# nateraw/stable-diffusion-videos

Hardware: AMD Instinct MI355X
Metric: interpolated frames/sec (512x512, 50 DDIM steps) (higher is better)
Workload: dtype bf16; 1 GPU; sd14 walk, 2 prompts, 640 interpolated frames (5 steps x 128 frames x 1 GPU; BASELINE config 2 names 60 frames - this is the same walk with more frames, see `walk_60_frames` for the literal one), 512x512, 50 DDIM steps, CFG 7.5; batch_size=128, frames=640, parallelism=frame-sharded dp1, hipgraph=True

## Files before the change

### include/sdv_hip.h

```cpp
#ifndef SDV_HIP_H
#define SDV_HIP_H

#include <stdint.h>

#ifdef __cplusplus
extern "C" {
#endif

typedef uint16_t sdv_bf16;

#define SDV_OK 0
#define SDV_ERR_ARG (-1)
#define SDV_ERR_LAUNCH (-2)

const char* sdv_last_error(void);
int sdv_abi_version(void);

typedef struct sdv_gemm_args {
    const sdv_bf16* X;
    const sdv_bf16* X2;
    const sdv_bf16* W;
    const float* bias;
    const sdv_bf16* R;
    sdv_bf16* C;
// ... 20 lines not shown
    uint8_t* out_u8;
    float* gn_out;
    int32_t gn_ld;
    int32_t split_k;
} sdv_gemm_args;

int sdv_gemm_bf16(const sdv_gemm_args* args, void* stream);
int sdv_gemm_stats_slots(const sdv_gemm_args* args);
int sdv_gemm_split_k(const sdv_gemm_args* args);

int sdv_gemm_set_persistent(int on);
int sdv_gemm_set_grid_limit(int n);
int sdv_rowstats_finalize(const float* partials, int64_t rows, int32_t slots, int32_t C, float eps, float* out, void* stream);

int sdv_ffn_geglu_bf16(const sdv_bf16* X, const float* ln_stats, int64_t M, int32_t C, int32_t ldx, const sdv_bf16* W1, const sdv_bf16* W1x,
                       const sdv_bf16* W2p, const float* bias2, sdv_bf16* out, int32_t ldo, void* stream);

int sdv_linear320_bf16(const sdv_bf16* X, int64_t M, int32_t ldx, const sdv_bf16* W, const sdv_bf16* Wx, int32_t N, const float* ln_stats,
                       const float* alpha, const sdv_bf16* R, int32_t ldr, sdv_bf16* out, int32_t ldo, float* stats_out, float eps,
                       sdv_bf16* Vt, int32_t ldvt, int32_t hw, void* stream);

int sdv_linear640_bf16(const sdv_bf16* X, int64_t M, int32_t ldx, const sdv_bf16* W, const sdv_bf16* Wx, int32_t N, const float* ln_stats,
                       const float* alpha, sdv_bf16* out, int32_t ldo, float* stats_out, float eps, void* stream);

int sdv_attention_bf16(const sdv_bf16* Q, const sdv_bf16* K, const sdv_bf16* Vt, sdv_bf16* O,
                       int32_t B, int32_t H, int32_t Lq, int32_t Lk, int32_t dh,
                       int32_t ldq, int32_t ldk, int32_t ldv, int32_t ldo, float scale, int32_t causal,
                       int32_t q_prescaled, int32_t v_rowmajor, void* stream);

int sdv_softmax_rows_bf16(sdv_bf16* S, int64_t rows, int32_t cols, int32_t ld, void* stream);
int sdv_softmax_rows_f32(const float* S, sdv_bf16* P, int64_t rows, int32_t cols, int32_t lds, int32_t ldp, void* stream);

int sdv_groupnorm_finalize(const float* P1, int32_t C1, int32_t ld1, int32_t bpi1, int32_t nrep1, int64_t rep_stride1,
                           const float* P2, int32_t C2, int32_t ld2, int32_t bpi2, int32_t nrep2, int64_t rep_stride2,
                           int32_t nimg, int32_t groups, int32_t splits, float* partials, void* stream);
int sdv_groupnorm_stats(const sdv_bf16* X, const sdv_bf16* X2, int32_t C1, int32_t C2, int32_t nimg,
                        int32_t HW, int32_t groups, int32_t splits, float* partials, void* stream);
int sdv_groupnorm_apply(const sdv_bf16* X, const sdv_bf16* X2, int32_t C1, int32_t C2, int32_t nimg,
                        int32_t HW, int32_t groups, int32_t splits, const float* partials,
                        const float* gamma, const float* beta, float eps, int32_t silu, sdv_bf16* Y,
                        void* stream);
int sdv_groupnorm_apply_fp8(const sdv_bf16* X, const sdv_bf16* X2, int32_t C1, int32_t C2, int32_t nimg,
                            int32_t HW, int32_t groups, int32_t splits, const float* partials,
                            const float* gamma, const float* beta, float eps, int32_t silu, uint8_t* Y8,
                            float q_scale, void* stream);
int sdv_groupnorm_fp8_set_saturation_counter(int32_t* counter);

int sdv_layernorm_bf16(const sdv_bf16* X, const float* gamma, const float* beta, float eps, int64_t rows,
                       int32_t C, sdv_bf16* Y, void* stream);

int sdv_conv3x3_cin_small(const sdv_bf16* X, const sdv_bf16* W , const float* bias,
                          sdv_bf16* Y, int32_t nimg, int32_t H, int32_t Wd, int32_t Cin, int32_t Cout,
                          int32_t circular, void* stream);
int sdv_im2col3x3_c4(const sdv_bf16* X, sdv_bf16* Y, int32_t nimg, int32_t H, int32_t Wd, int32_t circular, void* stream);

int sdv_latent_affine(const float* X, const float* Wpq , const float* bias, float in_scale,
                      sdv_bf16* Y, int64_t npix, int32_t C, void* stream);

int sdv_slerp_stats(const float* v0, const float* v1, int64_t n, double* stats, void* stream);
int sdv_slerp_batch(const float* v0, const float* v1, const double* stats, const float* T, int32_t nframes,
                    int32_t C, int32_t HW, int32_t to_hwc, float dot_threshold, float* out, void* stream);
int sdv_lerp_batch(const float* a, const float* b, const float* T, int32_t nframes, int64_t n,
                   float* out_f32, sdv_bf16* out_bf16, void* stream);

int sdv_cfg_ddim_step(const float* eps, float* latents, sdv_bf16* x2, const float* coefs,
                      const int32_t* step_ptr, const float* noise, float guidance, int32_t cfg,
                      int64_t n_per_batch , void* stream);
int sdv_cfg_multistep_step(const float* eps, float* latents, sdv_bf16* x2, float* hist, float* xsave, const float* table,
                           const int32_t* step_ptr, const float* noise, float guidance, int32_t cfg,
                           int64_t n_per_batch , void* stream);
int sdv_latents_to_unet_input(const float* latents, sdv_bf16* x2, int32_t cfg, int64_t n, void* stream);
int sdv_step_counter_add(int32_t* step_ptr, int32_t inc, void* stream);

int sdv_timestep_embedding(const float* timesteps, int32_t n, int32_t dim, int32_t flip_sin_to_cos,
                           float freq_shift, float* out, void* stream);
int sdv_linear_small(const float* x, const sdv_bf16* w, const float* b, const float* add, float* out,
                     int32_t M, int32_t N, int32_t K, int32_t silu_in, void* stream);

int sdv_nchw_to_nhwc_f32(const float* in, float* out, int32_t n, int32_t C, int32_t HW, void* stream);
int sdv_nhwc_to_nchw_f32(const float* in, float* out, int32_t n, int32_t C, int32_t HW, void* stream);
int sdv_f32_to_bf16(const float* in, sdv_bf16* out, int64_t n, void* stream);

int sdv_embed_tokens(const int64_t* ids, const float* tok , const float* pos , sdv_bf16* out,
                     int64_t n_tokens, int32_t L, int32_t D, int32_t vocab, void* stream);

int sdv_rgb_u8_to_bf16_c4(const uint8_t* in, sdv_bf16* out, int64_t npix, float scale, void* stream);
int sdv_axpby_bf16(const sdv_bf16* a, int32_t lda, const sdv_bf16* b, int32_t ldb, sdv_bf16* out, int32_t ldo,
                   int64_t rows, int32_t cols, float alpha, float beta, void* stream);

int sdv_clip_preprocess_patches(const uint8_t* frames, sdv_bf16* patches, int32_t n, int32_t H, int32_t W, int32_t S, int32_t P,
                                int32_t Kpad, const int32_t* x_off, const int32_t* x_cnt, const float* x_w, int32_t x_taps,
                                const int32_t* y_off, const int32_t* y_cnt, const float* y_w, int32_t y_taps,
                                const float* host_mean, const float* host_std, void* stream);
int sdv_safety_screen(const float* image_embeds, const float* concept_embeds, const float* special_care_embeds,
                      const float* concept_thr, const float* special_thr, int32_t n, int32_t D, int32_t n_concept,
                      int32_t n_special, uint8_t* frames, int64_t frame_bytes, int32_t* flags, float* scores, void* stream);

int sdv_jpeg_transform_u8(const uint8_t* frames, int32_t n, int32_t H, int32_t W, const uint16_t* qtab_luma,
                          const uint16_t* qtab_chroma, int16_t* coef, void* stream);
int sdv_jpeg_entropy_pack(const int16_t* coef, int32_t n, int32_t H, int32_t W, const uint8_t* header, int32_t header_len,
                          void* scratch, int64_t scratch_bytes, uint8_t* out, int64_t out_cap, int64_t* offsets, int64_t* needed,
                          void* stream);

int sdv_png_filter_u8(const uint8_t* frames, int32_t n, int32_t H, int32_t W, uint8_t* filtered, uint32_t* adler_rows, void* stream);
int sdv_png_deflate_pack(const uint8_t* filtered, const uint32_t* adler_rows, int32_t n, int32_t H, int32_t W, int32_t stripe_rows,
                         const uint8_t* header, int32_t header_len, void* scratch, int64_t scratch_bytes, uint8_t* out,
// ... 19 lines not shown
```

### stable_diffusion_videos_amd/build.py

```python
from __future__ import annotations

import os
import shutil
import subprocess
import sys
from concurrent.futures import ThreadPoolExecutor
from pathlib import Path

PKG = Path(__file__).resolve().parent
CSRC = PKG / "csrc"
INCLUDE = PKG.parent / "include"
LIBDIR = PKG / "lib"
OBJDIR = PKG / "lib" / "obj"
LIB = LIBDIR / "libsdv_hip.so"
ARCH = "gfx950"

FLAGS = ["--offload-arch=" + ARCH, "-O3", "-std=c++17", "-fPIC", "-Wno-unused-result", "-I", str(INCLUDE)]
FAST_MATH = {"sdv_gemm.hip", "sdv_attention.hip", "sdv_norm.hip", "sdv_ffn.hip"}
FAST_FLAGS = ["-ffast-math", "-fno-finite-math-only"]
EXTRA_FLAGS = {"sdv_attention.hip": ["-mllvm", "-amdgpu-mfma-vgpr-form"],
               "sdv_gemm.hip": ["-mllvm", "-amdgpu-mfma-vgpr-form", "-fno-slp-vectorize"],
               "sdv_ffn.hip": ["-fno-slp-vectorize"],
               "sdv_vision.hip": ["-fno-slp-vectorize"]}


def hipcc() -> str:
    exe = shutil.which("hipcc") or "/opt/rocm/bin/hipcc"
    if not Path(exe).exists():
        raise RuntimeError("hipcc not found: cannot build libsdv_hip.so")
    return exe


def sources():
    return sorted(CSRC.glob("*.hip"))


def _newest_dep() -> float:
    deps = list(CSRC.glob("*.h")) + list(INCLUDE.glob("*.h")) + [Path(__file__)]
    return max(p.stat().st_mtime for p in deps)


def _compile(src: Path, force: bool) -> Path:
    obj = OBJDIR / (src.stem + ".o")
    if (not force and obj.exists() and obj.stat().st_mtime >= src.stat().st_mtime
            and obj.stat().st_mtime >= _newest_dep()):
        return obj
    cmd = [hipcc(), *FLAGS, *(FAST_FLAGS if src.name in FAST_MATH else []), *EXTRA_FLAGS.get(src.name, []), "-c", str(src), "-o", str(obj)]
    r = subprocess.run(cmd, capture_output=True, text=True)
    if r.returncode != 0:
        raise RuntimeError(f"hipcc failed for {src.name}:\n{r.stdout}\n{r.stderr}")
    if r.stderr.strip():
        sys.stderr.write(r.stderr)
    return obj


def build(force: bool = False, verbose: bool = False) -> Path:
    OBJDIR.mkdir(parents=True, exist_ok=True)
    srcs = sources()
    if not srcs:
        raise RuntimeError(f"no .hip sources under {CSRC}")
    with ThreadPoolExecutor(max_workers=min(len(srcs), os.cpu_count() or 4)) as ex:
        objs = list(ex.map(lambda s: _compile(s, force), srcs))
    if force or not LIB.exists() or any(o.stat().st_mtime > LIB.stat().st_mtime for o in objs):
        cmd = [hipcc(), "--offload-arch=" + ARCH, "-shared", "-fPIC", *map(str, objs), "-o", str(LIB)]
        r = subprocess.run(cmd, capture_output=True, text=True)
        if r.returncode != 0:
            raise RuntimeError(f"link failed:\n{r.stdout}\n{r.stderr}")
    if verbose:
        print(f"built {LIB} ({LIB.stat().st_size >> 10} KiB) from {[s.name for s in srcs]}")
    return LIB


if __name__ == "__main__":
    build(force="--force" in sys.argv, verbose=True)
```

### stable_diffusion_videos_amd/csrc/sdv_norm.hip

```cpp
#include "sdv_common.h"

namespace {

struct GnGeom {
    int C, nchunk, CT, PT;
};
__device__ __forceinline__ GnGeom gn_geom(int C) {
    GnGeom g;
    g.C = C;
    g.nchunk = C >> 3;
    g.CT = g.nchunk < 256 ? g.nchunk : 256;
    g.PT = 256 / g.CT;
    return g;
}

__device__ __forceinline__ const uint16_t* gn_src(const uint16_t* X, const uint16_t* X2, int C1, int C2, long long pix,
                                                  int c0) {
    return c0 < C1 ? X + pix * C1 + c0 : X2 + pix * C2 + (c0 - C1);
}

__global__ __launch_bounds__(256) void gn_stats_kernel(const uint16_t* __restrict__ X, const uint16_t* __restrict__ X2,
                                                       int C1, int C2, int HW, int groups, int splits,
                                                       float* __restrict__ partials) {
    extern __shared__ __attribute__((aligned(16))) float sm[];
// ... 244 lines not shown
    const int sub = lane % LPR;
    const long long row = ((long long)blockIdx.x * 4 + (threadIdx.x >> 6)) * RPWV + lane / LPR;
    const bool live = row < rows;
    const uint16_t* x = X + (live ? row : 0) * C;
    bf16x8_raw raw[5];
#pragma unroll
    for (int i = 0; i < 5; ++i) raw[i] = *(const bf16x8_raw*)(x + (sub + LPR * i) * 8);
    float f[5][8];
    float s = 0.f;
#pragma unroll
    for (int i = 0; i < 5; ++i) {
        unpack8(raw[i], f[i]);
#pragma unroll
        for (int e = 0; e < 8; ++e) s += f[i][e];
    }
#pragma unroll
    for (int o = LPR / 2; o > 0; o >>= 1) s += __shfl_xor(s, o);
    const float mean = s / (float)C;
    float q = 0.f;
#pragma unroll
    for (int i = 0; i < 5; ++i)
#pragma unroll
        for (int e = 0; e < 8; ++e) {
            const float d = f[i][e] - mean;
            q += d * d;
        }
#pragma unroll
    for (int o = LPR / 2; o > 0; o >>= 1) q += __shfl_xor(q, o);
    const float rstd = rsqrtf(q / (float)C + eps);
    if (!live) return;
    uint16_t* y = Y + row * C;
#pragma unroll
    for (int i = 0; i < 5; ++i) {
        const int c0 = (sub + LPR * i) * 8;
        const float4 g0 = *(const float4*)(gamma + c0), g1 = *(const float4*)(gamma + c0 + 4);
        const float4 b0 = *(const float4*)(beta + c0), b1 = *(const float4*)(beta + c0 + 4);
        const float gg[8] = {g0.x, g0.y, g0.z, g0.w, g1.x, g1.y, g1.z, g1.w};
        const float bb[8] = {b0.x, b0.y, b0.z, b0.w, b1.x, b1.y, b1.z, b1.w};
        float o[8];
#pragma unroll
        for (int e = 0; e < 8; ++e) o[e] = (f[i][e] - mean) * rstd * gg[e] + bb[e];
        *(bf16x8_raw*)(y + c0) = pack8(o);
    }
}

}

namespace {
struct GnSrc {
    const float* P;
    int C, ld, bpi, nrep;
    long long rep_stride;
};
__global__ __launch_bounds__(256) void gn_finalize_kernel(GnSrc a, GnSrc b, int groups, int splits, float* __restrict__ partials) {
    extern __shared__ __attribute__((aligned(16))) float sm[];
    const int C = a.C + b.C, cpg = C / groups;
    const int img = blockIdx.x, split = blockIdx.y;
    for (int c = threadIdx.x; c < C; c += 256) {
        const GnSrc& s = c < a.C ? a : b;
        const int cc = c < a.C ? c : c - a.C;
        const int per = (s.bpi + splits - 1) / splits;
        const int k0 = split * per, k1 = k0 + per < s.bpi ? k0 + per : s.bpi;
        float s1 = 0.f, s2 = 0.f;
        for (int r = 0; r < s.nrep; ++r) {
            const float* base = s.P + ((r * s.rep_stride + (long long)img * s.bpi) * 2) * s.ld + cc;
            int k = k0;
            for (; k + 3 < k1; k += 4) {
                float t[8];
#pragma unroll
                for (int j = 0; j < 8; ++j) t[j] = base[(long long)(2 * k + j) * s.ld];
#pragma unroll
                for (int j = 0; j < 4; ++j) {
                    s1 += t[2 * j];
                    s2 += t[2 * j + 1];
                }
            }
            for (; k < k1; ++k) {
                s1 += base[(long long)(2 * k) * s.ld];
                s2 += base[(long long)(2 * k + 1) * s.ld];
            }
        }
        sm[2 * c] = s1;
        sm[2 * c + 1] = s2;
    }
    __syncthreads();
    if (threadIdx.x < groups) {
        float as = 0.f, aq = 0.f;
        for (int c = 0; c < cpg; ++c) {
            as += sm[2 * (threadIdx.x * cpg + c)];
            aq += sm[2 * (threadIdx.x * cpg + c) + 1];
        }
        float* out = partials + (((long long)img * splits + split) * groups + threadIdx.x) * 2;
        out[0] = as;
        out[1] = aq;
    }
}
}

extern "C" int sdv_groupnorm_finalize(const float* P1, int32_t C1, int32_t ld1, int32_t bpi1, int32_t nrep1, int64_t rep_stride1,
                                      const float* P2, int32_t C2, int32_t ld2, int32_t bpi2, int32_t nrep2, int64_t rep_stride2,
                                      int32_t nimg, int32_t groups, int32_t splits, float* partials, void* stream) {
    SDV_REQUIRE(P1 && partials && C1 > 0 && nimg > 0, "sdv_groupnorm_finalize: bad args");
    SDV_REQUIRE(C2 == 0 || P2, "sdv_groupnorm_finalize: C2 > 0 needs P2");
    const int C = C1 + C2;
    SDV_REQUIRE(groups > 0 && groups <= 64 && C % groups == 0, "sdv_groupnorm_finalize: bad groups %d for C=%d", groups, C);
    SDV_REQUIRE(bpi1 > 0 && nrep1 > 0 && (C2 == 0 || (bpi2 > 0 && nrep2 > 0)) && splits > 0 && splits <= 64, "sdv_groupnorm_finalize: bad block geometry");
    SDV_REQUIRE((size_t)C * 8 <= 64 * 1024, "sdv_groupnorm_finalize: C=%d too large", C);
    GnSrc a{P1, C1, ld1, bpi1, nrep1, rep_stride1};
    GnSrc b{C2 ? P2 : P1, C2, C2 ? ld2 : ld1, C2 ? bpi2 : 1, C2 ? nrep2 : 1, C2 ? rep_stride2 : 0};
    hipLaunchKernelGGL(gn_finalize_kernel, dim3(nimg, splits), dim3(256), (size_t)C * 8, (hipStream_t)stream, a, b, groups, splits, partials);
    SDV_CHECK_LAUNCH("sdv_groupnorm_finalize");
    return SDV_OK;
}

extern "C" int sdv_groupnorm_stats(const sdv_bf16* X, const sdv_bf16* X2, int32_t C1, int32_t C2, int32_t nimg,
                                   int32_t HW, int32_t groups, int32_t splits, float* partials, void* stream) {
    SDV_REQUIRE(X && partials, "sdv_groupnorm_stats: null pointer");
    SDV_REQUIRE(C2 == 0 || X2, "sdv_groupnorm_stats: C2 > 0 needs X2");
    const int C = C1 + C2;
    SDV_REQUIRE(C1 % 8 == 0 && C2 % 8 == 0 && C > 0, "sdv_groupnorm_stats: channels must be multiples of 8");
    SDV_REQUIRE(groups > 0 && groups <= 64 && C % groups == 0, "sdv_groupnorm_stats: bad groups %d for C=%d", groups, C);
    SDV_REQUIRE(splits > 0 && nimg > 0 && HW > 0, "sdv_groupnorm_stats: bad sizes");
    const int nchunk = C / 8;
    const int CT = nchunk < 256 ? nchunk : 256;
    const size_t lds = (size_t)(256 / CT) * C * 2 * sizeof(float);
    SDV_REQUIRE(lds <= 64 * 1024, "sdv_groupnorm_stats: C=%d too large", C);
    hipLaunchKernelGGL(gn_stats_kernel, dim3(splits, nimg), dim3(256), lds, (hipStream_t)stream, X, X2 ? X2 : X, C1, C2, HW,
                       groups, splits, partials);
    SDV_CHECK_LAUNCH("sdv_groupnorm_stats");
    return SDV_OK;
}

static int* g_fp8_sat_counter = nullptr;
extern "C" int sdv_groupnorm_fp8_set_saturation_counter(int32_t* counter) {
    g_fp8_sat_counter = counter;
    return SDV_OK;
}

static int gn_apply_launch(const sdv_bf16* X, const sdv_bf16* X2, int32_t C1, int32_t C2, int32_t nimg, int32_t HW,
                           int32_t groups, int32_t splits, const float* partials, const float* gamma, const float* beta,
                           float eps, int32_t silu, void* Y, bool fp8, float q_scale, void* stream) {
    SDV_REQUIRE(X && partials && gamma && beta && Y, "sdv_groupnorm_apply: null pointer");
    SDV_REQUIRE(C2 == 0 || X2, "sdv_groupnorm_apply: C2 > 0 needs X2");
    const int C = C1 + C2;
    SDV_REQUIRE(C1 % 8 == 0 && C2 % 8 == 0 && C > 0, "sdv_groupnorm_apply: channels must be multiples of 8");
    SDV_REQUIRE(groups > 0 && groups <= 64 && C % groups == 0, "sdv_groupnorm_apply: bad groups");
    SDV_REQUIRE(splits > 0 && nimg > 0 && HW > 0, "sdv_groupnorm_apply: bad sizes");
    long long ppb_elems = (long long)nimg * HW * C / 4096;
    ppb_elems = ppb_elems < 16384 ? 16384 : (ppb_elems > 131072 ? 131072 : ppb_elems);
    int ppb = (int)((ppb_elems + C - 1) / C);
    if (ppb < 1) ppb = 1;
    const int nblk = (HW + ppb - 1) / ppb;
    if (fp8)
        hipLaunchKernelGGL(gn_apply_kernel<true>, dim3(nblk, nimg), dim3(256), 0, (hipStream_t)stream, X, X2 ? X2 : X, C1, C2, HW,
                           groups, splits, partials, gamma, beta, eps, silu, ppb, (uint16_t*)Y, q_scale, g_fp8_sat_counter);
    else
        hipLaunchKernelGGL(gn_apply_kernel<false>, dim3(nblk, nimg), dim3(256), 0, (hipStream_t)stream, X, X2 ? X2 : X, C1, C2, HW,
                           groups, splits, partials, gamma, beta, eps, silu, ppb, (uint16_t*)Y, 1.0f, (int*)nullptr);
    SDV_CHECK_LAUNCH("sdv_groupnorm_apply");
    return SDV_OK;
}

extern "C" int sdv_groupnorm_apply(const sdv_bf16* X, const sdv_bf16* X2, int32_t C1, int32_t C2, int32_t nimg, int32_t HW,
// ... 70 lines not shown
```

### stable_diffusion_videos_amd/hip.py

```python
from __future__ import annotations

import ctypes as C
import os
from pathlib import Path
from typing import Optional

import torch

_LIB_PATH = Path(os.environ["SDV_HIP_LIB"]) if os.environ.get("SDV_HIP_LIB") else Path(__file__).resolve().parent / "lib" / "libsdv_hip.so"
_lib = None


class SdvHipError(RuntimeError):
    pass


class GemmArgs(C.Structure):
    _fields_ = [
        ("X", C.c_void_p), ("X2", C.c_void_p), ("W", C.c_void_p), ("bias", C.c_void_p), ("R", C.c_void_p),
        ("C", C.c_void_p), ("step_ptr", C.c_void_p), ("zero_page", C.c_void_p),
        ("sX", C.c_int64), ("sW", C.c_int64), ("sC", C.c_int64), ("sR", C.c_int64),
        ("M", C.c_int32), ("N", C.c_int32), ("K", C.c_int32),
        ("ldx", C.c_int32), ("ldx2", C.c_int32), ("C1", C.c_int32), ("ldw", C.c_int32), ("ldc", C.c_int32),
        ("ldr", C.c_int32),
        ("mode", C.c_int32), ("Hin", C.c_int32), ("Win", C.c_int32), ("Hout", C.c_int32), ("Wout", C.c_int32),
        ("circular", C.c_int32),
        ("epi", C.c_int32), ("bias_mode", C.c_int32), ("bias_step_stride", C.c_int32),
        ("batch", C.c_int32), ("tile", C.c_int32), ("alpha", C.c_float),
        ("div_hw_mul", C.c_uint32), ("div_hw_shr", C.c_uint32), ("div_w_mul", C.c_uint32), ("div_w_shr", C.c_uint32),
        ("alpha_cols", C.c_int32),
        ("ln_stats", C.c_void_p), ("ln_s", C.c_void_p), ("stats_out", C.c_void_p), ("ln_side", C.c_int32), ("stats_p", C.c_int32),
        ("fp8", C.c_int32), ("out_mode", C.c_int32), ("out_f32", C.c_void_p), ("out_u8", C.c_void_p),
        ("gn_out", C.c_void_p), ("gn_ld", C.c_int32), ("split_k", C.c_int32),
    ]


ABI_VERSION = 12


_SIGNATURES = {
    "sdv_last_error": (C.c_char_p, []),
    "sdv_abi_version": (C.c_int, []),
    "sdv_gemm_bf16": (C.c_int, [C.POINTER(GemmArgs), C.c_void_p]),
    "sdv_gemm_stats_slots": (C.c_int, [C.POINTER(GemmArgs)]),
    "sdv_gemm_split_k": (C.c_int, [C.POINTER(GemmArgs)]),
    "sdv_gemm_set_persistent": (C.c_int, [C.c_int]),
    "sdv_gemm_set_grid_limit": (C.c_int, [C.c_int]),
    "sdv_rowstats_finalize": (C.c_int, [C.c_void_p, C.c_int64, C.c_int32, C.c_int32, C.c_float, C.c_void_p, C.c_void_p]),
    "sdv_ffn_geglu_bf16": (C.c_int, [C.c_void_p, C.c_void_p, C.c_int64, C.c_int32, C.c_int32] + [C.c_void_p] * 5 + [C.c_int32, C.c_void_p]),
    "sdv_linear320_bf16": (C.c_int, [C.c_void_p, C.c_int64, C.c_int32, C.c_void_p, C.c_void_p, C.c_int32, C.c_void_p, C.c_void_p, C.c_void_p, C.c_int32,
                                     C.c_void_p, C.c_int32, C.c_void_p, C.c_float, C.c_void_p, C.c_int32, C.c_int32, C.c_void_p]),
    "sdv_linear640_bf16": (C.c_int, [C.c_void_p, C.c_int64, C.c_int32, C.c_void_p, C.c_void_p, C.c_int32, C.c_void_p, C.c_void_p, C.c_void_p, C.c_int32,
                                     C.c_void_p, C.c_float, C.c_void_p]),
    "sdv_attention_bf16": (C.c_int, [C.c_void_p] * 4 + [C.c_int32] * 9 + [C.c_float, C.c_int32, C.c_int32, C.c_int32, C.c_void_p]),
    "sdv_softmax_rows_bf16": (C.c_int, [C.c_void_p, C.c_int64, C.c_int32, C.c_int32, C.c_void_p]),
    "sdv_softmax_rows_f32": (C.c_int, [C.c_void_p, C.c_void_p, C.c_int64, C.c_int32, C.c_int32, C.c_int32, C.c_void_p]),
    "sdv_groupnorm_finalize": (C.c_int, ([C.c_void_p] + [C.c_int32] * 4 + [C.c_int64]) * 2 + [C.c_int32] * 3 + [C.c_void_p, C.c_void_p]),
    "sdv_groupnorm_stats": (C.c_int, [C.c_void_p, C.c_void_p] + [C.c_int32] * 6 + [C.c_void_p, C.c_void_p]),
    "sdv_groupnorm_apply": (C.c_int, [C.c_void_p, C.c_void_p] + [C.c_int32] * 6 + [C.c_void_p] * 3 +
                            [C.c_float, C.c_int32, C.c_void_p, C.c_void_p]),
    "sdv_groupnorm_apply_fp8": (C.c_int, [C.c_void_p, C.c_void_p] + [C.c_int32] * 6 + [C.c_void_p] * 3 +
                                [C.c_float, C.c_int32, C.c_void_p, C.c_float, C.c_void_p]),
    "sdv_groupnorm_fp8_set_saturation_counter": (C.c_int, [C.c_void_p]),
    "sdv_layernorm_bf16": (C.c_int, [C.c_void_p] * 3 + [C.c_float, C.c_int64, C.c_int32, C.c_void_p, C.c_void_p]),
    "sdv_conv3x3_cin_small": (C.c_int, [C.c_void_p] * 4 + [C.c_int32] * 6 + [C.c_void_p]),
    "sdv_im2col3x3_c4": (C.c_int, [C.c_void_p, C.c_void_p] + [C.c_int32] * 4 + [C.c_void_p]),
    "sdv_latent_affine": (C.c_int, [C.c_void_p] * 3 + [C.c_float, C.c_void_p, C.c_int64, C.c_int32, C.c_void_p]),
    "sdv_slerp_stats": (C.c_int, [C.c_void_p, C.c_void_p, C.c_int64, C.c_void_p, C.c_void_p]),
    "sdv_slerp_batch": (C.c_int, [C.c_void_p] * 4 + [C.c_int32] * 4 + [C.c_float, C.c_void_p, C.c_void_p]),
    "sdv_lerp_batch": (C.c_int, [C.c_void_p] * 3 + [C.c_int32, C.c_int64, C.c_void_p, C.c_void_p, C.c_void_p]),
    "sdv_cfg_ddim_step": (C.c_int, [C.c_void_p] * 6 + [C.c_float, C.c_int32, C.c_int64, C.c_void_p]),
    "sdv_cfg_multistep_step": (C.c_int, [C.c_void_p] * 8 + [C.c_float, C.c_int32, C.c_int64, C.c_void_p]),
    "sdv_latents_to_unet_input": (C.c_int, [C.c_void_p, C.c_void_p, C.c_int32, C.c_int64, C.c_void_p]),
    "sdv_step_counter_add": (C.c_int, [C.c_void_p, C.c_int32, C.c_void_p]),
    "sdv_timestep_embedding": (C.c_int, [C.c_void_p, C.c_int32, C.c_int32, C.c_int32, C.c_float, C.c_void_p,
                                         C.c_void_p]),
    "sdv_linear_small": (C.c_int, [C.c_void_p] * 5 + [C.c_int32] * 4 + [C.c_void_p]),
    "sdv_nchw_to_nhwc_f32": (C.c_int, [C.c_void_p, C.c_void_p, C.c_int32, C.c_int32, C.c_int32, C.c_void_p]),
    "sdv_nhwc_to_nchw_f32": (C.c_int, [C.c_void_p, C.c_void_p, C.c_int32, C.c_int32, C.c_int32, C.c_void_p]),
    "sdv_f32_to_bf16": (C.c_int, [C.c_void_p, C.c_void_p, C.c_int64, C.c_void_p]),
    "sdv_embed_tokens": (C.c_int, [C.c_void_p] * 4 + [C.c_int64, C.c_int32, C.c_int32, C.c_int32, C.c_void_p]),
    "sdv_rgb_u8_to_bf16_c4": (C.c_int, [C.c_void_p, C.c_void_p, C.c_int64, C.c_float, C.c_void_p]),
    "sdv_axpby_bf16": (C.c_int, [C.c_void_p, C.c_int32, C.c_void_p, C.c_int32, C.c_void_p, C.c_int32, C.c_int64, C.c_int32,
                                 C.c_float, C.c_float, C.c_void_p]),
    "sdv_clip_preprocess_patches": (C.c_int, [C.c_void_p, C.c_void_p] + [C.c_int32] * 6 + [C.c_void_p] * 3 + [C.c_int32] + [C.c_void_p] * 3 +
                                    [C.c_int32, C.POINTER(C.c_float), C.POINTER(C.c_float), C.c_void_p]),
    "sdv_safety_screen": (C.c_int, [C.c_void_p] * 5 + [C.c_int32] * 4 + [C.c_void_p, C.c_int64, C.c_void_p, C.c_void_p, C.c_void_p]),
    "sdv_jpeg_transform_u8": (C.c_int, [C.c_void_p] + [C.c_int32] * 3 + [C.POINTER(C.c_uint16), C.POINTER(C.c_uint16), C.c_void_p, C.c_void_p]),
    "sdv_jpeg_entropy_pack": (C.c_int, [C.c_void_p] + [C.c_int32] * 3 + [C.c_void_p, C.c_int32, C.c_void_p, C.c_int64, C.c_void_p, C.c_int64,
                                        C.c_void_p, C.c_void_p, C.c_void_p]),
    "sdv_png_filter_u8": (C.c_int, [C.c_void_p] + [C.c_int32] * 3 + [C.c_void_p, C.c_void_p, C.c_void_p]),
    "sdv_png_deflate_pack": (C.c_int, [C.c_void_p, C.c_void_p] + [C.c_int32] * 4 + [C.c_void_p, C.c_int32, C.c_void_p, C.c_int64, C.c_void_p, C.c_int64,
                                       C.c_void_p, C.c_void_p, C.c_void_p, C.c_void_p]),
    "sdv_png_deflate_lz_pack": (C.c_int, [C.c_void_p, C.c_void_p] + [C.c_int32] * 4 + [C.c_void_p, C.c_int32, C.c_void_p, C.c_int64, C.c_void_p,
                                          C.c_int64, C.c_void_p, C.c_void_p, C.c_void_p, C.c_void_p, C.c_int64, C.c_void_p, C.c_void_p,
                                          C.c_void_p]),
    "sdv_png_crc32": (C.c_int, [C.c_void_p, C.c_int64, C.c_void_p, C.c_void_p, C.c_int32, C.c_void_p, C.c_void_p]),
    "sdv_h264_planes_u8": (C.c_int, [C.c_void_p] + [C.c_int32] * 3 + [C.c_void_p] * 4),
# ... 47 lines not shown
        return None
    if not t.is_cuda:
        raise SdvHipError(f"{name} must live in GPU memory (got device {t.device}); the HIP path has no CPU fallback")
    if dtype is not None and t.dtype != dtype:
        raise SdvHipError(f"{name}: expected dtype {dtype}, got {t.dtype}")
    return t.data_ptr()


BF16 = torch.bfloat16
F32 = torch.float32
FP8 = torch.float8_e4m3fn
FP8_MAX = 448.0

_zero_pages = {}
FP8_MX = int(os.environ.get("SDV_FP8_MX", "1"))
FORCE_TILE = int(os.environ.get("SDV_FORCE_TILE", "0"))

LAUNCH_HOOK = None


def _launch(kind: str, info: dict, fn):
    if LAUNCH_HOOK is None:
        fn()
    else:
        LAUNCH_HOOK(kind, info, fn)


_OPLIB = torch.library.Library("sdv", "FRAGMENT")
KERNEL_OPS = []


def _defop(schema: str, impl, fake=None):
    name = schema[:schema.index("(")]
    _OPLIB.define(schema)
    _OPLIB.impl(name, impl, "CompositeExplicitAutograd")
    _OPLIB.impl(name, fake if fake is not None else (lambda *a, **k: None), "Meta")
    KERNEL_OPS.append(name)
    return getattr(torch.ops.sdv, name)


def zero_page(device) -> torch.Tensor:
    key = str(device)
    if key not in _zero_pages:
        _zero_pages[key] = torch.zeros(256, dtype=torch.uint8, device=device)
    return _zero_pages[key]


_GEMM_INTS = ("M", "N", "K", "ldx", "ldw", "ldc", "ldr", "C1", "ldx2", "epi", "mode", "Hin", "Win", "Hout", "Wout", "circular", "batch",
              "sX", "sW", "sC", "sR", "bias_mode", "bias_step_stride", "tile", "x_off", "w_off", "out_off", "alpha_cols", "out_mode")


GN_EPILOGUE = os.environ.get("SDV_GN_EPILOGUE", "1") != "0"
SPLIT_K = os.environ.get("SDV_SPLIT_K", "1") != "0"
LAST_SPLIT_K = 1


class GnStats:
    __slots__ = ("p", "C", "nimg", "HW", "bpi", "nrep", "rep_stride", "ver")

    def __init__(self, p, C, nimg, HW, bpi, nrep, rep_stride, ver=-1):
        self.p, self.C, self.nimg, self.HW, self.bpi, self.nrep, self.rep_stride, self.ver = p, C, nimg, HW, bpi, nrep, rep_stride, ver


def _ver(t: torch.Tensor) -> int:
    try:
        return t._version
    except RuntimeError:
        return -1


def gn_repeat(t_src: torch.Tensor, t_dst: torch.Tensor, times: int):
    g = getattr(t_src, "_sdv_gn", None)
    if g is not None and g.nrep == 1:
        t_dst._sdv_gn = GnStats(torch.cat([g.p] * times), g.C, g.nimg * times, g.HW, g.bpi, 1, 0, _ver(t_dst))


def gn_slice(t: torch.Tensor, first_img: int, n_img: int, HW: int) -> torch.Tensor:
    out = t[first_img * HW:(first_img + n_img) * HW]
    g = getattr(t, "_sdv_gn", None)
    if g is not None and g.HW == HW:
        if g.nrep == 1:
            p = g.p[first_img * g.bpi:(first_img + n_img) * g.bpi]
            out._sdv_gn = GnStats(p, g.C, n_img, HW, g.bpi, 1, 0, g.ver)
        else:
            p = g.p.view(g.nrep, g.rep_stride, 2, g.C)[:, first_img * g.bpi:(first_img + n_img) * g.bpi].contiguous()
            out._sdv_gn = GnStats(p.view(-1, 2, g.C), g.C, n_img, HW, g.bpi, g.nrep, n_img * g.bpi, g.ver)
    return out


def gn_join(parts, whole: torch.Tensor):
    gs = [getattr(t, "_sdv_gn", None) for t in parts]
    if gs and all(g is not None and g.nrep == 1 for g in gs):
        whole._sdv_gn = GnStats(torch.cat([g.p for g in gs]), gs[0].C, sum(g.nimg for g in gs), gs[0].HW, gs[0].bpi, 1, 0, _ver(whole))


def gn_epilogue_ok(*, M, N, epi, mode, ldc, ldr, out, bias, residual, fp8, ln, want_stats, out_mode, HW_out, batch, sC, sR) -> bool:
    if not GN_EPILOGUE or epi != 0 or out_mode or fp8 or ln is not None or want_stats or out is None:
        return False
    rows_per_image = HW_out // 4 if mode == 4 else HW_out
    if M % 32 or rows_per_image % 32 or N % 8 or ldc % 8 or (residual is not None and ldr % 8) or (sC | sR) % 8:
        return False
    ptrs = out.data_ptr() | (bias.data_ptr() if bias is not None else 0) | (residual.data_ptr() if residual is not None else 0)
    return ptrs % 16 == 0


def _igemm_impl(x, w, out, bias, residual, x2, ln_stats, ln_s, step_ptr, out_f32, out_u8, gn_out, ints, alpha, ln_eps, want_stats):
# ... 2 lines not shown
    lib = load()
    a = GemmArgs()
    fp8 = x.dtype == FP8
    if fp8:
        if w.dtype != FP8 or (x2 is not None and x2.dtype != FP8) or g["x_off"] or g["w_off"]:
            raise SdvHipError("gemm: fp8 activations need fp8 weights (and no operand offsets)")
        a.fp8 = 2 if FP8_MX else 1
        a.X, a.X2, a.W = _ptr(x, FP8, "X"), _ptr(x2, FP8, "X2"), _ptr(w, FP8, "W")
    else:
        a.X = _ptr(x, BF16, "X") + 2 * g["x_off"]
        a.X2 = _ptr(x2, BF16, "X2")
        a.W = _ptr(w, BF16, "W") + 2 * g["w_off"]
    a.bias = _ptr(bias, F32, "bias")
    a.R = _ptr(residual, BF16, "R")
    a.C = _ptr(out, BF16, "C") + 2 * g["out_off"] if out is not None else None
    a.out_mode, a.out_f32, a.out_u8 = g["out_mode"], _ptr(out_f32, F32, "out_f32"), _ptr(out_u8, torch.uint8, "out_u8")
    a.step_ptr = _ptr(step_ptr, torch.int32, "step_ptr")
    a.zero_page = zero_page(x.device).data_ptr()
    a.sX, a.sW, a.sC, a.sR = g["sX"], g["sW"], g["sC"], g["sR"]
    a.M, a.N, a.K = M, N, K
    a.ldx, a.ldx2, a.C1, a.ldw, a.ldc, a.ldr = g["ldx"], g["ldx2"], g["C1"], g["ldw"], g["ldc"], g["ldr"]
    a.mode, a.Hin, a.Win, a.Hout, a.Wout, a.circular = mode, g["Hin"], g["Win"], g["Hout"], g["Wout"], g["circular"]
    a.epi, a.bias_mode, a.bias_step_stride = epi, (g["bias_mode"] if bias is not None else 0), g["bias_step_stride"]
    a.batch, a.tile, a.alpha, a.alpha_cols = batch, g["tile"], alpha, g["alpha_cols"]
    if FORCE_TILE and not g["tile"] and not g["out_mode"] and epi < 3:
        a.tile = FORCE_TILE
    if ln_stats is not None:
        a.ln_stats, a.ln_s, a.ln_side = _ptr(ln_stats, F32, "ln_stats"), _ptr(ln_s, F32, "ln_s"), 1
    if gn_out is not None:
        a.gn_out, a.gn_ld = _ptr(gn_out, F32, "gn_out"), gn_out.shape[-1]
    split_used = False
    if (SPLIT_K and not fp8 and ln_stats is None and not want_stats and not g["out_mode"] and epi == 0 and batch <= 1 and mode != 4
            and out_f32 is None and not g["alpha_cols"] and M <= 4096 and K * (1 if mode == 0 else 9) >= 2048):
        a.split_k = 8
        S = lib.sdv_gemm_split_k(C.byref(a))
        if S > 1:
            ws = torch.empty((S, M, N), dtype=F32, device=x.device)
            a.out_f32, a.split_k = ws.data_ptr(), S
            split_used = True
        else:
            a.split_k = 0
    global LAST_SPLIT_K
    LAST_SPLIT_K = a.split_k if split_used else 1
    partials = None
    if want_stats:
        a.stats_out = 16
        slots = lib.sdv_gemm_stats_slots(C.byref(a))
        if slots <= 0:
            _check(-1, "sdv_gemm_stats_slots")
        partials = torch.empty((max(batch, 1) * M, slots, 2), dtype=F32, device=x.device)
        a.stats_out = partials.data_ptr()
    taps = 1 if mode == 0 else 9
    flops = 2.0 * M * N * K * taps * (4 if mode == 4 else batch)
    _launch("gemm" if mode == 0 else "conv3x3",
            dict(M=M * (4 if mode == 4 else 1), N=N, K=K * taps, batch=batch, flops=flops, mode=mode, epi=epi),
            lambda: _check(lib.sdv_gemm_bf16(C.byref(a), _stream()), "sdv_gemm_bf16"))
    if want_stats:
        nout = N // 2 if epi == 1 else N
        stats = torch.empty((max(batch, 1) * M, 2), dtype=F32, device=x.device)
        _launch("ln_stats", dict(bytes=8.0 * partials.shape[0] * (partials.shape[1] + 1)),
                lambda: _check(lib.sdv_rowstats_finalize(partials.data_ptr(), partials.shape[0], partials.shape[1], nout, ln_eps,
                                                         stats.data_ptr(), _stream()), "sdv_rowstats_finalize"))
        return stats
    return torch.empty(0, dtype=F32, device=x.device)


def _igemm_fake(x, w, out, bias, residual, x2, ln_stats, ln_s, step_ptr, out_f32, out_u8, gn_out, ints, alpha, ln_eps, want_stats):
    g = dict(zip(_GEMM_INTS, ints))
    return x.new_empty((max(g["batch"], 1) * g["M"], 2) if want_stats else (0,), dtype=F32)


_k_igemm = _defop("k_igemm(Tensor x, Tensor w, Tensor(a!)? out, Tensor? bias, Tensor? residual, Tensor? x2, Tensor? ln_stats, "
                  "Tensor? ln_s, Tensor? step_ptr, Tensor(b!)? out_f32, Tensor(c!)? out_u8, Tensor(d!)? gn_out, int[] ints, float alpha, "
                  "float ln_eps, bool want_stats) -> Tensor", _igemm_impl, _igemm_fake)


def gemm(x: torch.Tensor, w: torch.Tensor, out: torch.Tensor, *, M: int, N: int, K: int, ldx: int, ldw: int,
         ldc: int, bias: Optional[torch.Tensor] = None, bias_mode: int = 1, residual: Optional[torch.Tensor] = None,
         ldr: int = 0, x2: Optional[torch.Tensor] = None, C1: int = 0, ldx2: int = 0, alpha: float = 1.0,
         epi: int = 0, mode: int = 0, Hin: int = 0, Win: int = 0, Hout: int = 0, Wout: int = 0,
         circular: bool = False, batch: int = 1, sX: int = 0, sW: int = 0, sC: int = 0, sR: int = 0,
         step_ptr: Optional[torch.Tensor] = None, bias_step_stride: int = 0, tile: int = 0,
         x_off: int = 0, w_off: int = 0, out_off: int = 0, alpha_cols: int = 0, ln=None,
         want_stats: bool = False, ln_eps: float = 1e-5, out_mode: int = 0, out_f32: Optional[torch.Tensor] = None,
         out_u8: Optional[torch.Tensor] = None, gn_hw: int = 0):
    ints = [M, N, K, ldx, ldw, ldc, ldr, C1, ldx2, epi, mode, Hin, Win, Hout, Wout, int(circular), batch, sX, sW, sC, sR, bias_mode,
            bias_step_stride, tile, x_off, w_off, out_off, alpha_cols, out_mode]
    gn_out = None
    nb = max(batch, 1)
    if gn_hw and out_off == 0 and gn_epilogue_ok(M=M, N=N, epi=epi, mode=mode, ldc=ldc, ldr=ldr, out=out, bias=bias, residual=residual,
                                                 fp8=x.dtype == FP8, ln=ln, want_stats=want_stats, out_mode=out_mode, HW_out=gn_hw,
                                                 batch=batch, sC=sC, sR=sR):
        nrep = 4 if mode == 4 else 1
        rows = nb * M if mode != 4 else M
        gn_out = torch.empty((nrep * rows // 32, 2, N), dtype=F32, device=x.device)
    st = _k_igemm(x, w, out, bias, residual, x2, ln[0] if ln is not None else None, ln[1] if ln is not None else None, step_ptr,
                  out_f32, out_u8, gn_out, ints, float(alpha), float(ln_eps), bool(want_stats))
    if gn_out is not None:
        rows_per_image = gn_hw // 4 if mode == 4 else gn_hw
        nimg = (M if mode == 4 else nb * M) // rows_per_image
        out._sdv_gn = GnStats(gn_out, N, nimg, gn_hw, rows_per_image // 32, 4 if mode == 4 else 1, (M // 32) if mode == 4 else 0, _ver(out))
    elif out is not None and hasattr(out, "_sdv_gn"):
        del out._sdv_gn
    return st if want_stats else None


def linear(x: torch.Tensor, w: torch.Tensor, bias: Optional[torch.Tensor] = None, *, residual=None, out=None,
           epi: int = 0, x2: Optional[torch.Tensor] = None, alpha: float = 1.0, tile: int = 0, alpha_cols: int = 0, ln=None,
           want_stats: bool = False, ln_eps: float = 1e-5, gn_hw: int = 0):
# ... 1046 lines not shown
```

Baseline: 12.01 frames/s.

## Add direct conv3x3 kernel for narrow-output heads and widen GN finalize

Adds a dedicated direct 3x3 convolution kernel for convolutions with 1-4 output channels, such as the UNet conv_out to 4 latent channels and the VAE's final conv to RGB. It keeps all weights in LDS, stages a halo strip of input pixels, and accumulates with bf16 dot2 instructions instead of routing the op through the MFMA implicit GEMM, where N<=4 wastes most of the tile. The groupnorm finalize kernel is also changed to launch up to 1024 threads sized to C and to unroll its partial-sum loads 16 deep. Risks: the direct kernel's large LDS footprint limits occupancy, and the dot-product path may be slower than MFMA for large Cin.

```diff
diff --git a/include/sdv_hip.h b/include/sdv_hip.h
--- a/include/sdv_hip.h
+++ b/include/sdv_hip.h
@@ -96,6 +96,8 @@
 int sdv_conv3x3_cin_small(const sdv_bf16* X, const sdv_bf16* W , const float* bias,
                           sdv_bf16* Y, int32_t nimg, int32_t H, int32_t Wd, int32_t Cin, int32_t Cout,
                           int32_t circular, void* stream);
+int sdv_conv3x3_head_ok(const sdv_gemm_args* args);
+int sdv_conv3x3_head(const sdv_gemm_args* args, void* stream);
 int sdv_im2col3x3_c4(const sdv_bf16* X, sdv_bf16* Y, int32_t nimg, int32_t H, int32_t Wd, int32_t circular, void* stream);
 
 int sdv_latent_affine(const float* X, const float* Wpq , const float* bias, float in_scale,
diff --git a/stable_diffusion_videos_amd/build.py b/stable_diffusion_videos_amd/build.py
--- a/stable_diffusion_videos_amd/build.py
+++ b/stable_diffusion_videos_amd/build.py
@@ -21,6 +21,7 @@
 EXTRA_FLAGS = {"sdv_attention.hip": ["-mllvm", "-amdgpu-mfma-vgpr-form"],
                "sdv_gemm.hip": ["-mllvm", "-amdgpu-mfma-vgpr-form", "-fno-slp-vectorize"],
                "sdv_ffn.hip": ["-fno-slp-vectorize"],
+               "sdv_conv_head.hip": ["-fno-slp-vectorize"],
                "sdv_vision.hip": ["-fno-slp-vectorize"]}
 
 
diff --git a/stable_diffusion_videos_amd/csrc/sdv_conv_head.hip b/stable_diffusion_videos_amd/csrc/sdv_conv_head.hip
--- /dev/null
+++ b/stable_diffusion_videos_amd/csrc/sdv_conv_head.hip
@@ -0,0 +1,213 @@
+#include "sdv_common.h"
+
+namespace {
+
+constexpr int TR = 4, TC = 64;
+constexpr int SR = TR + 2, SC = TC + 2;
+constexpr int CK = 64;
+constexpr int PIX = 2 * CK + 16;
+constexpr int STRIP_BYTES = SR * SC * PIX;
+constexpr int NPIECE = SR * SC * (CK / 8);
+constexpr int NTHR = 256;
+constexpr int NIT = (NPIECE + NTHR - 1) / NTHR;
+constexpr int MAX_CIN = 1024;
+
+typedef __attribute__((ext_vector_type(2))) __bf16 bf16x2_t;
+
+struct HeadArgs {
+    const uint16_t* X;
+    const uint16_t* W;
+    const float* bias;
+    float* out_f32;
+    uint8_t* out_u8;
+    int H, Wd, Cin, ldx, ldw, ldc, out_mode, circular, tiles_x, tiles_y;
+};
+
+SDV_DEVICE float dot8(const uint4& a, const uint4& w, float acc) {
+    acc = __builtin_amdgcn_fdot2_f32_bf16(__builtin_bit_cast(bf16x2_t, a.x), __builtin_bit_cast(bf16x2_t, w.x), acc, false);
+    acc = __builtin_amdgcn_fdot2_f32_bf16(__builtin_bit_cast(bf16x2_t, a.y), __builtin_bit_cast(bf16x2_t, w.y), acc, false);
+    acc = __builtin_amdgcn_fdot2_f32_bf16(__builtin_bit_cast(bf16x2_t, a.z), __builtin_bit_cast(bf16x2_t, w.z), acc, false);
+    acc = __builtin_amdgcn_fdot2_f32_bf16(__builtin_bit_cast(bf16x2_t, a.w), __builtin_bit_cast(bf16x2_t, w.w), acc, false);
+    return acc;
+}
+
+template <int COUT>
+__global__ __launch_bounds__(NTHR) void conv_head_kernel(HeadArgs p) {
+    extern __shared__ __attribute__((aligned(16))) unsigned char smem[];
+    unsigned char* const wl = smem;
+    unsigned char* const strip = smem + COUT * 9 * p.Cin * 2;
+    const int tid = threadIdx.x, lane = tid & 63, wv = tid >> 6;
+    int t = blockIdx.x;
+    const int x0 = (t % p.tiles_x) * TC;
+    t /= p.tiles_x;
+    const int y0 = (t % p.tiles_y) * TR;
+    const int img = t / p.tiles_y;
+    const int H = p.H, Wd = p.Wd, Cin = p.Cin;
+
+    const int wrow = 9 * (Cin >> 3);
+    for (int i = tid; i < COUT * wrow; i += NTHR) {
+        const int co = i / wrow, k = i - co * wrow;
+        *(uint4*)(wl + (size_t)i * 16) = *(const uint4*)(p.W + (size_t)co * p.ldw + k * 8);
+    }
+
+    int src[NIT];
+#pragma unroll
+    for (int it = 0; it < NIT; ++it) {
+        const int j = tid + it * NTHR, pix = j >> 3;
+        const int ry = pix / SC, rx = pix - ry * SC;
+        int gy = y0 - 1 + ry, gx = x0 - 1 + rx;
+        if (p.circular) {
+            gy = gy < 0 ? gy + H : (gy >= H ? gy - H : gy);
+            gx = gx < 0 ? gx + Wd : (gx >= Wd ? gx - Wd : gx);
+        }
+        const bool in = j < NPIECE && gy >= 0 && gy < H && gx >= 0 && gx < Wd;
+        src[it] = in ? gy * Wd + gx : -1;
+    }
+    const uint16_t* const ximg = p.X + (size_t)img * H * Wd * p.ldx + (tid & 7) * 8;
+
+    float acc[TR][COUT];
+#pragma unroll
+    for (int r = 0; r < TR; ++r)
+#pragma unroll
+        for (int co = 0; co < COUT; ++co) acc[r][co] = 0.f;
+
+    for (int c0 = 0; c0 < Cin; c0 += CK) {
+        const int ng = Cin - c0 >= CK ? CK / 8 : (Cin - c0) >> 3;
+        uint4 v[NIT];
+#pragma unroll
+        for (int it = 0; it < NIT; ++it) {
+            v[it] = make_uint4(0u, 0u, 0u, 0u);
+            if (src[it] >= 0 && (tid & 7) < ng) v[it] = *(const uint4*)(ximg + (size_t)src[it] * p.ldx + c0);
+        }
+        __syncthreads();
+#pragma unroll
+        for (int it = 0; it < NIT; ++it) {
+            const int j = tid + it * NTHR;
+            if (j < NPIECE) *(uint4*)(strip + (j >> 3) * PIX + (j & 7) * 16) = v[it];
+        }
+        __syncthreads();
+        for (int g = wv; g < ng; g += 4) {
+            const unsigned char* const wg = wl + (size_t)(c0 + g * 8) * 2;
+            const unsigned char* const ag = strip + lane * PIX + g * 16;
+#pragma unroll
+            for (int dx = 0; dx < 3; ++dx) {
+                uint4 w[3][COUT];
+#pragma unroll
+                for (int dy = 0; dy < 3; ++dy)
+#pragma unroll
+                    for (int co = 0; co < COUT; ++co) w[dy][co] = *(const uint4*)(wg + (size_t)((co * 9 + dy * 3 + dx) * Cin) * 2);
+#pragma unroll
+                for (int ry = 0; ry < SR; ++ry) {
+                    const uint4 a = *(const uint4*)(ag + (ry * SC + dx) * PIX);
+#pragma unroll
+                    for (int dy = 0; dy < 3; ++dy) {
+                        const int r = ry - dy;
+                        if (r >= 0 && r < TR) {
+#pragma unroll
+                            for (int co = 0; co < COUT; ++co) acc[r][co] = dot8(a, w[dy][co], acc[r][co]);
+                        }
+                    }
+                }
+            }
+        }
+    }
+
+    __syncthreads();
+    float* const red = (float*)strip;
+#pragma unroll
+    for (int r = 0; r < TR; ++r)
+#pragma unroll
+        for (int co = 0; co < COUT; ++co) red[((wv * TR + r) * COUT + co) * 64 + lane] = acc[r][co];
+    __syncthreads();
+    const int y = y0 + wv, x = x0 + lane;
+    if (y >= H || x >= Wd) return;
+    float o[COUT];
+#pragma unroll
+    for (int co = 0; co < COUT; ++co) {
+        float s = red[((0 * TR + wv) * COUT + co) * 64 + lane];
+#pragma unroll
+        for (int k = 1; k < 4; ++k) s += red[((k * TR + wv) * COUT + co) * 64 + lane];
+        o[co] = p.bias ? s + p.bias[co] : s;
+    }
+    const size_t idx = ((size_t)(img * H + y) * Wd + x) * p.ldc;
+    if (p.out_mode == 1) {
+        if (COUT == 4 && (p.ldc & 3) == 0 && (((uintptr_t)p.out_f32) & 15) == 0) {
+            *(float4*)(p.out_f32 + idx) = make_float4(o[0], o[1], o[2], o[COUT - 1]);
+        } else {
+#pragma unroll
+            for (int co = 0; co < COUT; ++co) p.out_f32[idx + co] = o[co];
+        }
+    } else {
+#pragma unroll
+        for (int co = 0; co < COUT; ++co) {
+            const float tt = fminf(fmaxf(o[co] * 0.5f + 0.5f, 0.f), 1.f);
+            if (p.out_f32) p.out_f32[idx + co] = tt;
+            if (p.out_u8) p.out_u8[idx + co] = (uint8_t)rintf(tt * 255.0f);
+        }
+    }
+}
+
+bool head_form(const sdv_gemm_args& a) {
+    if (a.mode != 1 || a.N < 1 || a.N > 4 || (a.out_mode != 1 && a.out_mode != 2)) return false;
+    if (a.R || a.epi != 0 || a.ln_side || a.ln_stats || a.stats_out || a.gn_out || a.fp8 || a.batch > 1 || a.split_k > 1 || a.tile != 0) return false;
+    if ((a.alpha != 1.f && a.alpha != 0.f) || a.alpha_cols || a.step_ptr || (a.bias && a.bias_mode == 2)) return false;
+    if (a.X2 && a.X2 != a.X) return false;
+    if (!a.X || !a.W || a.K <= 0 || a.K % 8 || a.K > MAX_CIN || a.ldx % 8 || a.ldw % 8 || a.ldx < a.K || a.ldw < 9 * a.K) return false;
+    if ((((uintptr_t)a.X | (uintptr_t)a.W) & 15) || (((uintptr_t)a.bias | (uintptr_t)a.out_f32) & 3)) return false;
+    if (a.Hin <= 0 || a.Win <= 0 || a.Hin != a.Hout || a.Win != a.Wout || a.M <= 0 || a.M % (a.Hin * a.Win) || a.ldc < a.N) return false;
+    if (a.out_mode == 1 ? !a.out_f32 : (!a.out_f32 && !a.out_u8)) return false;
+    const long long tiles = (long long)(a.M / (a.Hin * a.Win)) * ((a.Hin + TR - 1) / TR) * ((a.Win + TC - 1) / TC);
+    return tiles <= 0x7fffffffLL;
+}
+
+template <int COUT>
+void head_launch(const HeadArgs& p, dim3 grid, size_t lds, hipStream_t s) {
+    static unsigned long long attr_set = 0;
+    int dev = 0;
+    (void)hipGetDevice(&dev);
+    const unsigned long long dev_bit = 1ull << (dev & 63);
+    if (!(attr_set & dev_bit)) {
+        (void)hipFuncSetAttribute((const void*)conv_head_kernel<COUT>, hipFuncAttributeMaxDynamicSharedMemorySize,
+                                  COUT * 9 * MAX_CIN * 2 + STRIP_BYTES);
+        attr_set |= dev_bit;
+    }
+    hipLaunchKernelGGL(conv_head_kernel<COUT>, grid, dim3(NTHR), lds, s, p);
+}
+
+}
+
+extern "C" int sdv_conv3x3_head_ok(const sdv_gemm_args* args) { return args != nullptr && head_form(*args) ? 1 : 0; }
+
+extern "C" int sdv_conv3x3_head(const sdv_gemm_args* args, void* stream) {
+    SDV_REQUIRE(args != nullptr, "sdv_conv3x3_head: null args");
+    const sdv_gemm_args& a = *args;
+    SDV_REQUIRE(head_form(a), "sdv_conv3x3_head: not a launch of the direct form (ask sdv_conv3x3_head_ok first)");
+    HeadArgs p;
+    p.X = (const uint16_t*)a.X;
+    p.W = (const uint16_t*)a.W;
+    p.bias = a.bias;
+    p.out_f32 = a.out_f32;
+    p.out_u8 = a.out_u8;
+    p.H = a.Hin;
+    p.Wd = a.Win;
+    p.Cin = a.K;
+    p.ldx = a.ldx;
+    p.ldw = a.ldw;
+    p.ldc = a.ldc;
+    p.out_mode = a.out_mode;
+    p.circular = a.circular;
+    p.tiles_x = (a.Win + TC - 1) / TC;
+    p.tiles_y = (a.Hin + TR - 1) / TR;
+    const int nimg = a.M / (a.Hin * a.Win);
+    const dim3 grid((unsigned)(nimg * p.tiles_y * p.tiles_x));
+    const size_t lds = (size_t)a.N * 9 * a.K * 2 + STRIP_BYTES;
+    hipStream_t s = (hipStream_t)stream;
+    switch (a.N) {
+        case 1: head_launch<1>(p, grid, lds, s); break;
+        case 2: head_launch<2>(p, grid, lds, s); break;
+        case 3: head_launch<3>(p, grid, lds, s); break;
+        default: head_launch<4>(p, grid, lds, s); break;
+    }
+    SDV_CHECK_LAUNCH("sdv_conv3x3_head");
+    return SDV_OK;
+}
diff --git a/stable_diffusion_videos_amd/csrc/sdv_norm.hip b/stable_diffusion_videos_amd/csrc/sdv_norm.hip
--- a/stable_diffusion_videos_amd/csrc/sdv_norm.hip
+++ b/stable_diffusion_videos_amd/csrc/sdv_norm.hip
@@ -320,32 +320,44 @@
     int C, ld, bpi, nrep;
     long long rep_stride;
 };
-__global__ __launch_bounds__(256) void gn_finalize_kernel(GnSrc a, GnSrc b, int groups, int splits, float* __restrict__ partials) {
+__global__ __launch_bounds__(1024) void gn_finalize_kernel(GnSrc a, GnSrc b, int groups, int splits, float* __restrict__ partials) {
+#pragma clang fp reassociate(off)
     extern __shared__ __attribute__((aligned(16))) float sm[];
     const int C = a.C + b.C, cpg = C / groups;
     const int img = blockIdx.x, split = blockIdx.y;
-    for (int c = threadIdx.x; c < C; c += 256) {
+    for (int c = threadIdx.x; c < C; c += blockDim.x) {
         const GnSrc& s = c < a.C ? a : b;
         const int cc = c < a.C ? c : c - a.C;
         const int per = (s.bpi + splits - 1) / splits;
         const int k0 = split * per, k1 = k0 + per < s.bpi ? k0 + per : s.bpi;
+        const long long ld = s.ld;
         float s1 = 0.f, s2 = 0.f;
         for (int r = 0; r < s.nrep; ++r) {
-            const float* base = s.P + ((r * s.rep_stride + (long long)img * s.bpi) * 2) * s.ld + cc;
+            const float* q = s.P + ((r * s.rep_stride + (long long)img * s.bpi + k0) * 2) * ld + cc;
             int k = k0;
+            for (; k + 15 < k1; k += 16) {
+                float t[32];
+#pragma unroll
+                for (int j = 0; j < 32; ++j, q += ld) t[j] = *q;
+#pragma unroll
+                for (int j = 0; j < 16; ++j) {
+                    s1 += t[2 * j];
+                    s2 += t[2 * j + 1];
+                }
+            }
             for (; k + 3 < k1; k += 4) {
                 float t[8];
 #pragma unroll
-                for (int j = 0; j < 8; ++j) t[j] = base[(long long)(2 * k + j) * s.ld];
+                for (int j = 0; j < 8; ++j, q += ld) t[j] = *q;
 #pragma unroll
                 for (int j = 0; j < 4; ++j) {
                     s1 += t[2 * j];
                     s2 += t[2 * j + 1];
                 }
             }
-            for (; k < k1; ++k) {
-                s1 += base[(long long)(2 * k) * s.ld];
-                s2 += base[(long long)(2 * k + 1) * s.ld];
+            for (; k < k1; ++k, q += 2 * ld) {
+                s1 += q[0];
+                s2 += q[ld];
             }
         }
         sm[2 * c] = s1;
@@ -376,7 +388,8 @@
     SDV_REQUIRE((size_t)C * 8 <= 64 * 1024, "sdv_groupnorm_finalize: C=%d too large", C);
     GnSrc a{P1, C1, ld1, bpi1, nrep1, rep_stride1};
     GnSrc b{C2 ? P2 : P1, C2, C2 ? ld2 : ld1, C2 ? bpi2 : 1, C2 ? nrep2 : 1, C2 ? rep_stride2 : 0};
-    hipLaunchKernelGGL(gn_finalize_kernel, dim3(nimg, splits), dim3(256), (size_t)C * 8, (hipStream_t)stream, a, b, groups, splits, partials);
+    const int threads = C >= 1024 ? 1024 : (C + 63) / 64 * 64;
+    hipLaunchKernelGGL(gn_finalize_kernel, dim3(nimg, splits), dim3(threads), (size_t)C * 8, (hipStream_t)stream, a, b, groups, splits, partials);
     SDV_CHECK_LAUNCH("sdv_groupnorm_finalize");
     return SDV_OK;
 }
diff --git a/stable_diffusion_videos_amd/hip.py b/stable_diffusion_videos_amd/hip.py
--- a/stable_diffusion_videos_amd/hip.py
+++ b/stable_diffusion_videos_amd/hip.py
@@ -44,6 +44,8 @@
     "sdv_gemm_bf16": (C.c_int, [C.POINTER(GemmArgs), C.c_void_p]),
     "sdv_gemm_stats_slots": (C.c_int, [C.POINTER(GemmArgs)]),
     "sdv_gemm_split_k": (C.c_int, [C.POINTER(GemmArgs)]),
+    "sdv_conv3x3_head_ok": (C.c_int, [C.POINTER(GemmArgs)]),
+    "sdv_conv3x3_head": (C.c_int, [C.POINTER(GemmArgs), C.c_void_p]),
     "sdv_gemm_set_persistent": (C.c_int, [C.c_int]),
     "sdv_gemm_set_grid_limit": (C.c_int, [C.c_int]),
     "sdv_rowstats_finalize": (C.c_int, [C.c_void_p, C.c_int64, C.c_int32, C.c_int32, C.c_float, C.c_void_p, C.c_void_p]),
@@ -197,6 +199,7 @@
 
 GN_EPILOGUE = os.environ.get("SDV_GN_EPILOGUE", "1") != "0"
 SPLIT_K = os.environ.get("SDV_SPLIT_K", "1") != "0"
+CONV_HEAD_DIRECT = os.environ.get("SDV_CONV_HEAD_DIRECT", "1") != "0"
 LAST_SPLIT_K = 1
 
 
@@ -305,9 +308,12 @@
         a.stats_out = partials.data_ptr()
     taps = 1 if mode == 0 else 9
     flops = 2.0 * M * N * K * taps * (4 if mode == 4 else batch)
+    if CONV_HEAD_DIRECT and mode == 1 and g["out_mode"] and lib.sdv_conv3x3_head_ok(C.byref(a)):
+        run = lambda: _check(lib.sdv_conv3x3_head(C.byref(a), _stream()), "sdv_conv3x3_head")
+    else:
+        run = lambda: _check(lib.sdv_gemm_bf16(C.byref(a), _stream()), "sdv_gemm_bf16")
     _launch("gemm" if mode == 0 else "conv3x3",
-            dict(M=M * (4 if mode == 4 else 1), N=N, K=K * taps, batch=batch, flops=flops, mode=mode, epi=epi),
-            lambda: _check(lib.sdv_gemm_bf16(C.byref(a), _stream()), "sdv_gemm_bf16"))
+            dict(M=M * (4 if mode == 4 else 1), N=N, K=K * taps, batch=batch, flops=flops, mode=mode, epi=epi), run)
     if want_stats:
         nout = N // 2 if epi == 1 else N
         stats = torch.empty((max(batch, 1) * M, 2), dtype=F32, device=x.device)
```

After: 12.05 frames/s, median of 6. No clear change (+0.4%).
